# petim0/fly_bProject

Hardware: AMD Instinct MI355X
Metric: env-steps/sec (PPO rollout + update), 8192 envs per GPU (higher is better)
Workload: dtype f32 (optimizer step: fp16x2 operand split; rollout policy + critic: bf16x3 operand split; fp32 accumulate)

## Files before the change

### fly_bproject_amd/csrc/domain_rand.h

```cpp
#ifndef DOMAIN_RAND_H
#define DOMAIN_RAND_H

#include "flyhip.h"
#include "obs_norm.h"

struct DrSlot {
    float* table;
    FlyRandomization r;
};
constexpr unsigned long DR_SLOT = OBS_NORM_SLOT + 16;
constexpr unsigned long DR_CONFIG_BYTES = DR_SLOT + ((sizeof(DrSlot) + 15) & ~15UL);
static_assert(FLY_DR_PARAMS == 6 && FLY_DR_ROW == 8, "a row is m[6] | count | 0: two 16-byte stores");

#ifdef __HIPCC__
__device__ __forceinline__ const DrSlot* dr_slot(const FlyConfig* c)
{
    return reinterpret_cast<const DrSlot*>(reinterpret_cast<const char*>(c) + DR_SLOT);
}

__device__ __forceinline__ uint32_t dr_lowbias32(uint32_t x)
{
    x ^= x >> 16;
    x *= 0x7feb352du;
    x ^= x >> 15;
    x *= 0x846ca68bu;
    x ^= x >> 16;
    return x;
}

__device__ __forceinline__ void dr_draw(const FlyConfig* c, uint32_t e, uint32_t k, float m[FLY_DR_PARAMS])
{
    const DrSlot* s = dr_slot(c);
    const uint32_t key = dr_lowbias32(s->r.seed ^ dr_lowbias32(e));
    const uint32_t ctr = dr_lowbias32(key + k);
#pragma unroll
    for (int j = 0; j < FLY_DR_PARAMS; ++j) {
        const uint32_t h = dr_lowbias32(ctr + 0x9E3779B9u * (uint32_t)(j + 1));
        const float u = __fmul_rn((float)(h >> 8), 5.9604644775390625e-8f);
        const float lo = s->r.lo[j], hi = s->r.hi[j];
        m[j] = __fadd_rn(lo, __fmul_rn(__fsub_rn(hi, lo), u));
    }
}

__device__ __forceinline__ void dr_load_row(const FlyConfig* c, long e, float m[FLY_DR_PARAMS], uint32_t& k)
{
    const float4* row = reinterpret_cast<const float4*>(dr_slot(c)->table + e * FLY_DR_ROW);
    const float4 a = row[0], b = row[1];
    m[0] = a.x; m[1] = a.y; m[2] = a.z; m[3] = a.w; m[4] = b.x; m[5] = b.y;
    k = __builtin_bit_cast(uint32_t, b.z);
}

__device__ __forceinline__ void dr_store_row(const FlyConfig* c, long e, const float m[FLY_DR_PARAMS], uint32_t k)
{
    float4* row = reinterpret_cast<float4*>(dr_slot(c)->table + e * FLY_DR_ROW);
    row[0] = make_float4(m[0], m[1], m[2], m[3]);
    row[1] = make_float4(m[4], m[5], __builtin_bit_cast(float, k), 0.0f);
}
#endif

#endif
```

### fly_bproject_amd/csrc/fly_body.inc

```

constexpr int LANES_PER_ENV = 8;
constexpr int BLOCK = 256;
constexpr int ENVS_PER_BLOCK = BLOCK / LANES_PER_ENV;


template <int CTRL>
__device__ __forceinline__ float dpp_f(float x)
{
    return __builtin_bit_cast(float, __builtin_amdgcn_update_dpp(0, __builtin_bit_cast(int, x), CTRL, 0xF, 0xF, true));
}
template <int CTRL>
__device__ __forceinline__ int dpp_i(int x)
{
    return __builtin_amdgcn_update_dpp(0, x, CTRL, 0xF, 0xF, true);
}
__device__ __forceinline__ float row_sum(float x)
{
    x += dpp_f<0xB1>(x);
    x += dpp_f<0x4E>(x);
    x += dpp_f<0x141>(x);
    return x;
}
__device__ __forceinline__ int row_sum_i(int x)
{
    x += dpp_i<0xB1>(x);
    x += dpp_i<0x4E>(x);
    x += dpp_i<0x141>(x);
    return x;
}
__device__ __forceinline__ float row_get(float x, int src)
{
    return __shfl(x, src, LANES_PER_ENV);
}

__device__ __forceinline__ float dot3(float a0, float a1, float a2, float b0, float b1, float b2)
{
    return fmaf(a0, b0, fmaf(a1, b1, a2 * b2));
}
__device__ __forceinline__ float clampf(float x, float lim) { return fminf(fmaxf(x, -lim), lim); }

struct Root {
    float px, py, pz, qx, qy, qz, qw, vx, vy, vz, wx, wy, wz;
};

__device__ __forceinline__ void quat_rot(const float q[4], float v0, float v1, float v2, float sign, float o[3])
{
    float qw = q[3];
    float s = 2.0f * (qw * qw) - 1.0f;
    float cx = q[1] * v2 - q[2] * v1;
    float cy = q[2] * v0 - q[0] * v2;
    float cz = q[0] * v1 - q[1] * v0;
    float dot = q[0] * v0 + q[1] * v1 + q[2] * v2;
    o[0] = (v0 * s + sign * (cx * qw * 2.0f)) + q[0] * dot * 2.0f;
    o[1] = (v1 * s + sign * (cy * qw * 2.0f)) + q[1] * dot * 2.0f;
    o[2] = (v2 * s + sign * (cz * qw * 2.0f)) + q[2] * dot * 2.0f;
}

__device__ __forceinline__ float py_mod(float a, float b)
{
    float m = fmodf(a, b);
    if (m != 0.0f && ((b < 0.0f) != (m < 0.0f))) m += b;
    return m;
}

struct RootObs {
    float vl[3], wl[3], yaw, roll, pitch, ang, up_proj, heading_proj, pot;
};

__device__ __forceinline__ RootObs root_obs(const FlyConfig* __restrict__ c, const Root& r)
{
    RootObs o;
    const float two_pi = 6.28318530717958647692f;
    float t0 = c->target[0] - r.px, t1 = c->target[1] - r.py, t2 = 0.0f;
    float nrm = sqrtf(t0 * t0 + t1 * t1 + t2 * t2);
    o.pot = -nrm / c->dt;
    float dn = nrm < 1e-9f ? 1e-9f : nrm;
    float d0 = t0 / dn, d1 = t1 / dn, d2 = t2 / dn;
    float x1 = r.qx, y1 = r.qy, z1 = r.qz, w1 = r.qw;
    float x2 = -0.0f, y2 = -0.0f, z2 = -0.0f, w2 = 1.0f;
    float ww = (z1 + x1) * (x2 + y2);
    float yy = (w1 - y1) * (w2 + z2);
    float zz = (w1 + y1) * (w2 - z2);
    float xx = ww + yy + zz;
    float qq = 0.5f * (xx + (z1 - x1) * (x2 - y2));
    float tq[4];
    tq[3] = qq - ww + (z1 - y1) * (y2 - z2);
    tq[0] = qq - xx + (x1 + w1) * (x2 + w2);
    tq[1] = qq - yy + (w1 - x1) * (y2 + z2);
    tq[2] = qq - zz + (z1 + y1) * (w2 - x2);
    float up[3], hd[3];
    quat_rot(tq, 0.0f, 0.0f, 1.0f, 1.0f, up);
    quat_rot(tq, 1.0f, 0.0f, 0.0f, 1.0f, hd);
    o.up_proj = up[2];
    o.heading_proj = hd[0] * d0 + hd[1] * d1 + hd[2] * d2;
    quat_rot(tq, r.vx, r.vy, r.vz, -1.0f, o.vl);
    quat_rot(tq, r.wx, r.wy, r.wz, -1.0f, o.wl);
    float x = tq[0], y = tq[1], z = tq[2], w = tq[3];
    float sinr = 2.0f * (w * x + y * z);
    float cosr = w * w - x * x - y * y + z * z;
    float roll = atan2f(sinr, cosr);
    float sinp = 2.0f * (w * y - z * x);
    float pitch;
    if (fabsf(sinp) >= 1.0f) {
        float sgn = (sinp > 0.0f) ? 1.0f : ((sinp < 0.0f) ? -1.0f : 0.0f);
        pitch = 1.57079632679489661923f * sgn;
    } else {
        pitch = asinf(sinp);
    }
    float siny = 2.0f * (w * z + x * y);
    float cosy = w * w + x * x - y * y - z * z;
    float yaw = atan2f(siny, cosy);
    o.roll = py_mod(roll, two_pi);
    o.pitch = py_mod(pitch, two_pi);
    o.yaw = py_mod(yaw, two_pi);
    float walk = atan2f(c->target[2] - r.pz, c->target[0] - r.px);
    o.ang = walk - o.yaw;
    return o;
}

__device__ __forceinline__ float scale_action(float a, float lo, float hi)
{
    float t = 0.5f * (a + 1.0f);
    t = t * (hi - lo);
    return t + lo;
}

struct FlyRegs {
    Root r;
    float jq[3], jqd[3];
    float pot, prev_pot;
    int rs;
    long progress;
    float dm[FLY_DR_PARAMS];
    uint32_t dk;
};

template <int PH, bool DR = false>
__device__ __forceinline__ void fly_load(FlyRegs& st, const FlyConfig* __restrict__ c, const FlyBuffers& b, const int block)
{
    const int n = c->num_envs;
    const int tid = threadIdx.x;
    const int sub = tid & (LANES_PER_ENV - 1);
    const long e_raw = (long)block * ENVS_PER_BLOCK + tid / LANES_PER_ENV;
    const long e = e_raw < n ? e_raw : (long)(n - 1);
    const bool is_leg = sub < FLY_NUM_LEGS;
    const int j0 = 3 * (is_leg ? sub : 0);
    constexpr bool NEED_ROOT = (PH & (PH_RESET | PH_INTEGRATE | PH_OBS | PH_REWARD)) != 0;
    constexpr bool NEED_DOF = (PH & (PH_RESET | PH_INTEGRATE | PH_OBS)) != 0;
    constexpr bool NEED_POT = (PH & (PH_RESET | PH_OBS | PH_REWARD)) != 0;
    constexpr bool NEED_FLAG = (PH & (PH_RESET | PH_REWARD)) != 0;
    constexpr bool NEED_PROG = (PH & (PH_RESET | PH_REWARD | PH_PROGRESS)) != 0;
    Root r = {};
    if (NEED_ROOT) {
        const float* rp = b.root + e * FLY_ROOT_DIM;
        r.px = rp[0]; r.py = rp[1]; r.pz = rp[2]; r.qx = rp[3]; r.qy = rp[4]; r.qz = rp[5]; r.qw = rp[6];
        r.vx = rp[7]; r.vy = rp[8]; r.vz = rp[9]; r.wx = rp[10]; r.wy = rp[11]; r.wz = rp[12];
    }
    st.r = r;
#pragma unroll
    for (int i = 0; i < 3; ++i) { st.jq[i] = 0.0f; st.jqd[i] = 0.0f; }
    if (NEED_DOF && is_leg) {
        const float* dp = b.dof_state + e * (FLY_NUM_DOF * 2) + 2 * j0;
#pragma unroll
        for (int i = 0; i < 3; ++i) { st.jq[i] = dp[2 * i]; st.jqd[i] = dp[2 * i + 1]; }
    }
    st.pot = 0.0f; st.prev_pot = 0.0f;
    if (NEED_POT) { st.pot = b.pot[e]; st.prev_pot = b.prev_pot[e]; }
    st.rs = 0;
    if (NEED_FLAG) st.rs = (int)(b.reset[e] != 0);
    st.progress = 0;
    if (NEED_PROG) st.progress = b.progress[e];
    if constexpr (DR && (PH & (PH_RESET | PH_INTEGRATE)) != 0) dr_load_row(c, e, st.dm, st.dk);
}

template <int PH, bool DR = false>
__device__ __forceinline__ void fly_body(const FlyConfig* __restrict__ c, const float* __restrict__ actions, const FlyBuffers& b,
                                         float* obs_tile, const int block, const FlyRegs& st, FlyRegs* st_out = nullptr,
                                         const float* actions_tile = nullptr)
{

    const int n = c->num_envs;
    const int tid = threadIdx.x;
    const int sub = tid & (LANES_PER_ENV - 1);
    const int env_in_blk = tid / LANES_PER_ENV;
    const long e_raw = (long)block * ENVS_PER_BLOCK + env_in_blk;
    const bool valid = e_raw < n;
    const long e = valid ? e_raw : (long)(n - 1);
    const bool is_leg = sub < FLY_NUM_LEGS;
    const bool is_abd = sub < FLY_NUM_ABDOMEN;
    const int leg = is_leg ? sub : 0;
    const int abd = is_abd ? sub : 0;
    const int j0 = 3 * leg;

    float lo[3], hi[3], pose[3];
#pragma unroll
    for (int i = 0; i < 3; ++i) { lo[i] = c->dof_lo[j0 + i]; hi[i] = c->dof_hi[j0 + i]; pose[i] = c->dof_pose[j0 + i]; }

    Root r = st.r;
    float jq[3] = {st.jq[0], st.jq[1], st.jq[2]}, jqd[3] = {st.jqd[0], st.jqd[1], st.jqd[2]}, jt[3] = {0, 0, 0};
    float pot = st.pot, prev_pot = st.prev_pot;
    int rs = st.rs;
    long progress = st.progress;
    float dm[FLY_DR_PARAMS];
    uint32_t dk = 0;
    bool drew = false;
    if constexpr (DR) {
#pragma unroll
        for (int j = 0; j < FLY_DR_PARAMS; ++j) dm[j] = st.dm[j];
        dk = st.dk;
    }
    float cf[3] = {0, 0, 0};
    float cfa[3] = {0, 0, 0};

    if (PH & PH_SCALE) {
        if (is_leg) {
            const float* ap = actions_tile ? actions_tile + env_in_blk * FLY_NUM_DOF + j0 : actions + e * FLY_NUM_DOF + j0;
#pragma unroll
            for (int i = 0; i < 3; ++i) jt[i] = scale_action(ap[i], lo[i], hi[i]);
        }
    } else if ((PH & (PH_INTEGRATE | PH_OBS | PH_REWARD)) && is_leg) {
        const float* tp = b.targets + e * FLY_NUM_DOF + j0;
#pragma unroll
        for (int i = 0; i < 3; ++i) jt[i] = tp[i];
    }
    if (!(PH & (PH_INTEGRATE)) && (PH & (PH_OBS | PH_REWARD))) {
        if (is_leg) {
            const float* fp = b.contact + (e * FLY_NUM_CONTACT + FLY_NUM_ABDOMEN + leg) * 3;
            cf[0] = fp[0]; cf[1] = fp[1]; cf[2] = fp[2];
        }
        if (is_abd) {
            const float* fp = b.contact + (e * FLY_NUM_CONTACT + abd) * 3;
            cfa[0] = fp[0]; cfa[1] = fp[1]; cfa[2] = fp[2];
        }
    }

    const bool reset_after = c->reset_after_sim != 0;

    auto do_reset = [&]() {
        if (rs) {
            r.px = 0.0f; r.py = 0.0f; r.pz = c->start_height; r.qx = 0.0f; r.qy = 0.0f; r.qz = 0.0f; r.qw = 1.0f;
            r.vx = r.vy = r.vz = r.wx = r.wy = r.wz = 0.0f;
#pragma unroll
            for (int i = 0; i < 3; ++i) { jq[i] = is_leg ? pose[i] : 0.0f; jqd[i] = 0.0f; }
            float tx = c->target[0] - 0.0f, ty = c->target[1] - 0.0f;
            float nrm = sqrtf(__fadd_rn(__fadd_rn(__fmul_rn(tx, tx), __fmul_rn(ty, ty)), 0.0f));
            float p = -nrm / c->dt;
            prev_pot = p; pot = p;
            rs = 0; progress = 0;
            if constexpr (DR) {
                dr_draw(c, (uint32_t)e, dk, dm);
                dk += 1u;
                drew = true;
            }
        }
    };

    if ((PH & PH_RESET) && !(reset_after && (PH & PH_INTEGRATE))) do_reset();

    if (PH & PH_INTEGRATE) {
        const int nsub = c->substeps;
        const float h = c->dt / (float)nsub;
        const float kp = DR ? __fmul_rn(c->kp, dm[0]) : c->kp, kd = DR ? __fmul_rn(c->kd, dm[1]) : c->kd;
        const float eff = DR ? __fmul_rn(c->effort, dm[2]) : c->effort, vmax = c->vmax, Jinv = 1.0f / c->joint_inertia;
        const float minv = 1.0f / (DR ? __fmul_rn(c->mass, dm[3]) : c->mass), g = DR ? __fmul_rn(c->gravity, dm[5]) : c->gravity;
        const float I0 = DR ? __fmul_rn(c->inertia[0], dm[3]) : c->inertia[0];
        const float I1 = DR ? __fmul_rn(c->inertia[1], dm[3]) : c->inertia[1];
        const float I2 = DR ? __fmul_rn(c->inertia[2], dm[3]) : c->inertia[2];
        const float I0inv = 1.0f / I0, I1inv = 1.0f / I1, I2inv = 1.0f / I2;
        const float vlim = c->max_lin_vel, wlim = c->max_ang_vel;
        const float kc = c->kc, cd = c->cdamp, mu = DR ? __fmul_rn(c->mu, dm[4]) : c->mu, cv = c->cvisc;
        const float Lf = c->femur_len, Lt = c->tibia_len;
        const float ld = 1.0f - h * c->lin_damp, ad = 1.0f - h * c->ang_damp;
        const float att0 = c->leg_attach[leg][0], att1 = c->leg_attach[leg][1], att2 = c->leg_attach[leg][2];
        const float azim = c->leg_azimuth[leg], sg = c->leg_sigma[leg];
        const float ab0 = c->abdomen_pts[abd][0], ab1 = c->abdomen_pts[abd][1], ab2 = c->abdomen_pts[abd][2];
        const float al0 = c->alpha0, be0 = c->beta0;
        const float kc_leg = is_leg ? kc : 0.0f, kc_abd = is_abd ? kc : 0.0f;

        for (int s = 0; s < nsub; ++s) {
#pragma unroll
            for (int i = 0; i < 3; ++i) {
                float tau = fmaf(kp, jt[i] - jq[i], -(kd * jqd[i]));
                tau = fminf(fmaxf(tau, -eff), eff);
                float v = fmaf(h * Jinv, tau, jqd[i]);
                v = fminf(fmaxf(v, -vmax), vmax);
                float x = fmaf(h, v, jq[i]);
                if (x < lo[i]) { x = lo[i]; v = fmaxf(v, 0.0f); }
                if (x > hi[i]) { x = hi[i]; v = fminf(v, 0.0f); }
                jq[i] = x; jqd[i] = v;
            }
            const float qx = r.qx, qy = r.qy, qz = r.qz, qw = r.qw;
            const float R00 = fmaf(-2.0f, fmaf(qy, qy, qz * qz), 1.0f), R01 = 2.0f * fmaf(qx, qy, -(qz * qw)), R02 = 2.0f * fmaf(qx, qz, qy * qw);
            const float R10 = 2.0f * fmaf(qx, qy, qz * qw), R11 = fmaf(-2.0f, fmaf(qx, qx, qz * qz), 1.0f), R12 = 2.0f * fmaf(qy, qz, -(qx * qw));
            const float R20 = 2.0f * fmaf(qx, qz, -(qy * qw)), R21 = 2.0f * fmaf(qy, qz, qx * qw), R22 = fmaf(-2.0f, fmaf(qx, qx, qy * qy), 1.0f);
            float psi = fmaf(sg, jq[0] - pose[0], azim);
            float al = al0 + (jq[1] - pose[1]);
            float gm = al + be0 + (jq[2] - pose[2]);
            float psid = sg * jqd[0], ald = jqd[1], gmd = ald + jqd[2];
            const float sp = __sinf(psi), cp = __cosf(psi);
            const float sa = __sinf(al), ca = __cosf(al);
            const float sgm = __sinf(gm), cg = __cosf(gm);
            float rho = fmaf(Lf, ca, Lt * cg), zeta = fmaf(Lf, sa, Lt * sgm);
            float rhod = -fmaf(Lf * sa, ald, Lt * sgm * gmd);
            float zetad = fmaf(Lf * ca, ald, Lt * cg * gmd);
            float Fx_l = 0.0f, Fy_l = 0.0f, Fz_l = 0.0f, Tx_l = 0.0f, Ty_l = 0.0f, Tz_l = 0.0f;
            auto contact = [&](float rbx, float rby, float rbz, float rdx, float rdy, float rdz, float kc_l, auto moving, float (&f)[3]) {
                constexpr bool MOVING = decltype(moving)::value;
                float rwx = dot3(R00, R01, R02, rbx, rby, rbz);
                float rwy = dot3(R10, R11, R12, rbx, rby, rbz);
                float rwz = dot3(R20, R21, R22, rbx, rby, rbz);
                float d = fmaxf(-(r.pz + rwz), 0.0f);
                float ux = r.vx + fmaf(r.wy, rwz, -(r.wz * rwy));
                float uy = r.vy + fmaf(r.wz, rwx, -(r.wx * rwz));
                float uz = r.vz + fmaf(r.wx, rwy, -(r.wy * rwx));
                if (MOVING) {
                    ux += dot3(R00, R01, R02, rdx, rdy, rdz);
                    uy += dot3(R10, R11, R12, rdx, rdy, rdz);
                    uz += dot3(R20, R21, R22, rdx, rdy, rdz);
                }
                float fn = fmaxf(kc_l * d * fmaf(-cd, uz, 1.0f), 0.0f);
                float ut = __builtin_amdgcn_sqrtf(fmaf(ux, ux, uy * uy));
                float ft = fminf(cv * ut, mu * fn);
                float sc = ft * __builtin_amdgcn_rcpf(ut + 1e-9f);
                float fx = -sc * ux, fy = -sc * uy, fz = fn;
                f[0] = fx; f[1] = fy; f[2] = fz;
                Fx_l += fx; Fy_l += fy; Fz_l += fz;
                Tx_l += fmaf(rwy, fz, -(rwz * fy));
                Ty_l += fmaf(rwz, fx, -(rwx * fz));
                Tz_l += fmaf(rwx, fy, -(rwy * fx));
            };
            contact(fmaf(cp, rho, att0), fmaf(sp, rho, att1), att2 + zeta,
                    fmaf(cp, rhod, -(sp * rho * psid)), fmaf(sp, rhod, cp * rho * psid), zetad, kc_leg, std::true_type{}, cf);
            contact(ab0, ab1, ab2, 0.0f, 0.0f, 0.0f, kc_abd, std::false_type{}, cfa);
            float Fx = row_sum(Fx_l), Fy = row_sum(Fy_l), Fz = row_sum(Fz_l);
            float Tx = row_sum(Tx_l), Ty = row_sum(Ty_l), Tz = row_sum(Tz_l);
            r.vx = clampf(fmaf(h, Fx * minv, r.vx) * ld, vlim);
            r.vy = clampf(fmaf(h, Fy * minv, r.vy) * ld, vlim);
            r.vz = clampf(fmaf(h, fmaf(Fz, minv, g), r.vz) * ld, vlim);
            float wbx = dot3(R00, R10, R20, r.wx, r.wy, r.wz);
            float wby = dot3(R01, R11, R21, r.wx, r.wy, r.wz);
            float wbz = dot3(R02, R12, R22, r.wx, r.wy, r.wz);
            float tbx = dot3(R00, R10, R20, Tx, Ty, Tz);
            float tby = dot3(R01, R11, R21, Tx, Ty, Tz);
            float tbz = dot3(R02, R12, R22, Tx, Ty, Tz);
            float ax = (tbx - fmaf(wby * I2, wbz, -(wbz * I1 * wby))) * I0inv;
            float ay = (tby - fmaf(wbz * I0, wbx, -(wbx * I2 * wbz))) * I1inv;
            float az = (tbz - fmaf(wbx * I1, wby, -(wby * I0 * wbx))) * I2inv;
            wbx = clampf(fmaf(h, ax, wbx) * ad, wlim);
            wby = clampf(fmaf(h, ay, wby) * ad, wlim);
            wbz = clampf(fmaf(h, az, wbz) * ad, wlim);
            r.wx = dot3(R00, R01, R02, wbx, wby, wbz);
            r.wy = dot3(R10, R11, R12, wbx, wby, wbz);
            r.wz = dot3(R20, R21, R22, wbx, wby, wbz);
            r.px = fmaf(h, r.vx, r.px); r.py = fmaf(h, r.vy, r.py); r.pz = fmaf(h, r.vz, r.pz);
            const float hh = 0.5f * h;
            float nqx = fmaf(hh, fmaf(r.wx, qw, fmaf(r.wy, qz, -(r.wz * qy))), qx);
            float nqy = fmaf(hh, fmaf(-r.wx, qz, fmaf(r.wy, qw, r.wz * qx)), qy);
            float nqz = fmaf(hh, fmaf(r.wx, qy, fmaf(-r.wy, qx, r.wz * qw)), qz);
            float nqw = fmaf(hh, -fmaf(r.wx, qx, fmaf(r.wy, qy, r.wz * qz)), qw);
            float inv = __builtin_amdgcn_rsqf(fmaf(nqx, nqx, fmaf(nqy, nqy, fmaf(nqz, nqz, nqw * nqw))));
            r.qx = nqx * inv; r.qy = nqy * inv; r.qz = nqz * inv; r.qw = nqw * inv;
        }
    }

    if ((PH & PH_RESET) && reset_after && (PH & PH_INTEGRATE)) do_reset();

    float touching_f = 0.0f;
    float obs_act[3] = {0, 0, 0};
    float z_obs = 0.0f, heading_proj = 0.0f;
    if (PH & PH_OBS) {
        prev_pot = pot;
        RootObs ro = root_obs(c, r);
        pot = ro.pot;
        float* row = obs_tile + env_in_blk * FLY_NUM_OBS;
        if (sub == LANES_PER_ENV - 1) {
            row[0] = r.pz; row[1] = ro.vl[0]; row[2] = ro.vl[1]; row[3] = ro.vl[2];
            row[4] = ro.wl[0]; row[5] = ro.wl[1]; row[6] = ro.wl[2];
            row[7] = ro.yaw; row[8] = ro.roll; row[9] = ro.ang; row[10] = ro.up_proj; row[11] = ro.heading_proj;
            row[66] = ro.pitch;
        }
        z_obs = r.pz; heading_proj = ro.heading_proj;
        if (is_leg) {
            const float vs = c->dof_vel_scale;
#pragma unroll
            for (int i = 0; i < 3; ++i) {
                float u = __fsub_rn(__fsub_rn(__fmul_rn(2.0f, jq[i]), hi[i]), lo[i]) / __fsub_rn(hi[i], lo[i]);
                row[12 + j0 + i] = u;
                row[30 + j0 + i] = __fmul_rn(jqd[i], vs);
                row[48 + j0 + i] = jt[i];
                obs_act[i] = jt[i];
            }
            float ssum = __fadd_rn(__fadd_rn(cf[0], cf[1]), cf[2]);
            touching_f = ssum > 0.0f ? 1.0f : 0.0f;
            row[67 + leg] = touching_f;
        }
        __syncthreads();
        const long tile_base = (long)block * ENVS_PER_BLOCK * FLY_NUM_OBS;
        const long total = (long)n * FLY_NUM_OBS;
        const float4* src4 = reinterpret_cast<const float4*>(obs_tile);
        const bool aligned16 = (reinterpret_cast<uintptr_t>(b.obs) & 15) == 0;
        for (int i = tid; i < ENVS_PER_BLOCK * FLY_NUM_OBS / 4; i += BLOCK) {
            long g = tile_base + 4L * i;
            if (aligned16 && g + 3 < total) {
                *reinterpret_cast<float4*>(b.obs + g) = src4[i];
            } else {
                for (int k = 0; k < 4; ++k)
                    if (g + k < total) b.obs[g + k] = obs_tile[4 * i + k];
            }
        }
    } else if (PH & PH_REWARD) {
        const float* row = b.obs + e * FLY_NUM_OBS;
        z_obs = row[0]; heading_proj = row[11];
        if (is_leg) {
#pragma unroll
            for (int i = 0; i < 3; ++i) obs_act[i] = row[48 + j0 + i];
        }
    }

    if (PH & PH_PROGRESS) progress += 1;

    float reward = 0.0f;
    if (PH & PH_REWARD) {
        if (progress == 0) progress = 1;
        const float uw = c->up_weight, hw = c->heading_weight;
        float elec = 0.0f, acost = 0.0f;
        int lim = 0, touching = 0;
        if (is_leg) {
#pragma unroll
            for (int i = 0; i < 3; ++i) {
                acost += jt[i] * jt[i];
                elec += fabsf(__fsub_rn(jt[i], obs_act[i]));
                lim += (obs_act[i] > __fmul_rn(hi[i], 0.9f)) ? 1 : 0;
                lim += (obs_act[i] < __fmul_rn(lo[i], 0.9f)) ? 1 : 0;
            }
            touching = (__fadd_rn(__fadd_rn(cf[0], cf[1]), cf[2]) > 0.0f) ? 1 : 0;
        }
        elec = row_sum(elec); acost = row_sum(acost);
        lim = row_sum_i(lim); touching = row_sum_i(touching);
        float bsum = is_abd ? __fadd_rn(__fadd_rn(cfa[0], cfa[1]), cfa[2]) : 0.0f;
        float abd_sum = 0.0f;
#pragma unroll
        for (int k = 0; k < FLY_NUM_ABDOMEN; ++k) abd_sum = __fadd_rn(abd_sum, row_get(bsum, k));
        const float z = z_obs;
        float heading_r = (heading_proj > 0.8f) ? hw : __fmul_rn(hw, heading_proj) / 0.8f;
        float up_r = 0.0f;
        if (z > 1.4f) up_r = __fadd_rn(up_r, uw);
        if (z < 2.1f) up_r = __fsub_rn(up_r, uw);
        float ori = __fadd_rn(__fmul_rn(r.qz, r.qz), __fmul_rn(r.qw, r.qw));
        float orient_r = (ori > 0.98f) ? uw : 0.0f;
        float leg_r = __fmul_rn((float)touching, 0.1f);
        float progress_r = __fsub_rn(pot, prev_pot);
        float total;
        if (c->reward_mode == 0) {
            total = __fadd_rn(0.5f, __fmul_rn(up_r, orient_r));
            total = __fsub_rn(total, __fmul_rn(c->energy_cost_scale, elec));
            total = __fsub_rn(total, __fmul_rn((float)lim, c->joints_at_limit_cost_scale));
            total = __fadd_rn(total, leg_r);
        } else {
            total = __fadd_rn(__fmul_rn(progress_r, 2.0f), 0.5f);
            total = __fadd_rn(total, __fmul_rn(up_r, orient_r));
            total = __fadd_rn(total, heading_r);
            total = __fsub_rn(total, __fmul_rn(c->actions_cost_scale, acost));
            total = __fsub_rn(total, __fmul_rn(c->energy_cost_scale, elec));
            total = __fsub_rn(total, __fmul_rn((float)lim, c->joints_at_limit_cost_scale));
        }
        const bool dead = (z < c->termination_height) || (z > c->termination_height_up) || (ori < 0.5f) || (abd_sum > 0.0f);
        if (dead) total = c->death_cost;
        if (dead || progress >= (long)c->max_episode_length - 1) rs = 1;
        reward = total;
    }

    if (st_out) {
        st_out->r = r;
#pragma unroll
        for (int i = 0; i < 3; ++i) { st_out->jq[i] = jq[i]; st_out->jqd[i] = jqd[i]; }
        st_out->pot = pot; st_out->prev_pot = prev_pot; st_out->rs = rs; st_out->progress = progress;
        if constexpr (DR) {
#pragma unroll
            for (int j = 0; j < FLY_DR_PARAMS; ++j) st_out->dm[j] = dm[j];
            st_out->dk = dk;
        }
    }
    if (!valid) return;
    if constexpr (DR) {
        if (drew && sub == 0) dr_store_row(c, e, dm, dk);
    }
    if (PH & (PH_SCALE)) {
        if (is_leg) {
            float* tp = b.targets + e * FLY_NUM_DOF + j0;
#pragma unroll
            for (int i = 0; i < 3; ++i) tp[i] = jt[i];
        }
    }
    if (PH & (PH_RESET | PH_INTEGRATE)) {
        if (is_leg) {
            float* dp = b.dof_state + e * (FLY_NUM_DOF * 2) + 2 * j0;
#pragma unroll
            for (int i = 0; i < 3; ++i) { dp[2 * i] = jq[i]; dp[2 * i + 1] = jqd[i]; }
        }
        if (sub == LANES_PER_ENV - 1) {
            float* rp = b.root + e * FLY_ROOT_DIM;
            rp[0] = r.px; rp[1] = r.py; rp[2] = r.pz; rp[3] = r.qx; rp[4] = r.qy; rp[5] = r.qz; rp[6] = r.qw;
            rp[7] = r.vx; rp[8] = r.vy; rp[9] = r.vz; rp[10] = r.wx; rp[11] = r.wy; rp[12] = r.wz;
        }
    }
    if (PH & PH_INTEGRATE) {
        if (is_leg) {
            float* fp = b.contact + (e * FLY_NUM_CONTACT + FLY_NUM_ABDOMEN + leg) * 3;
            fp[0] = cf[0]; fp[1] = cf[1]; fp[2] = cf[2];
        }
        if (is_abd) {
            float* fp = b.contact + (e * FLY_NUM_CONTACT + abd) * 3;
            fp[0] = cfa[0]; fp[1] = cfa[1]; fp[2] = cfa[2];
        }
    }
    if (sub == LANES_PER_ENV - 2) {
        if (PH & (PH_RESET | PH_OBS)) { b.pot[e] = pot; b.prev_pot[e] = prev_pot; }
        if (PH & (PH_RESET | PH_REWARD)) b.reset[e] = (int64_t)rs;
        if (PH & (PH_RESET | PH_REWARD | PH_PROGRESS)) b.progress[e] = (int64_t)progress;
        if (PH & PH_REWARD) {
            b.reward[e] = reward;
            if (b.ep_return) {
                const float er = b.ep_return[e] + reward, el = b.ep_length[e] + 1.0f;
                if (rs) {
                    b.done_return[e] += er; b.done_length[e] += el; b.done_count[e] += 1.0f;
                    b.ep_return[e] = 0.0f; b.ep_length[e] = 0.0f;
                } else {
                    b.ep_return[e] = er; b.ep_length[e] = el;
                }
            }
        }
    }
}
// ... 1 lines not shown
```

### fly_bproject_amd/csrc/flyhip_abi.hip

```cpp
#include <hip/hip_runtime.h>
#include <string.h>
#include <stdint.h>
#include <stdio.h>
#include <stdarg.h>
#include <new>
#include "flyhip.h"
#include "obs_norm.h"
#include "domain_rand.h"
#include "launch.h"
#include <math.h>

struct FlyEnv {
    FlyConfig host;
    FlyConfig* dev;
    float* poses;
    const float* obs_norm;
    float* dr_table;
};

namespace {
thread_local char g_err[512] = "";

int fail(int code, const char* fmt, ...)
{
// ... 4 lines not shown
    return code;
}

int hip_fail(hipError_t e, const char* what)
{
    return fail(FLY_E_HIP, "%s: %s", what, hipGetErrorString(e));
}

int check_buffers(const FlyBuffers* b, int phases)
{
    if (!b) return fail(FLY_E_ARG, "FlyBuffers is null");
    const bool need_root = phases & (PH_RESET | PH_INTEGRATE | PH_OBS | PH_REWARD);
    const bool need_dof = phases & (PH_RESET | PH_INTEGRATE | PH_OBS);
    const bool need_tgt = phases & (PH_SCALE | PH_INTEGRATE | PH_OBS | PH_REWARD);
    const bool need_con = phases & (PH_INTEGRATE | PH_OBS | PH_REWARD);
    const bool need_pot = phases & (PH_RESET | PH_OBS | PH_REWARD);
    const bool need_obs = phases & (PH_OBS | PH_REWARD);
    const bool need_flags = phases & (PH_RESET | PH_REWARD | PH_PROGRESS);
    if (need_root && !b->root) return fail(FLY_E_ARG, "root is null");
    if (need_dof && !b->dof_state) return fail(FLY_E_ARG, "dof_state is null");
    if (need_tgt && !b->targets) return fail(FLY_E_ARG, "targets is null");
    if (need_con && !b->contact) return fail(FLY_E_ARG, "contact is null");
    if (need_pot && (!b->pot || !b->prev_pot)) return fail(FLY_E_ARG, "pot/prev_pot is null");
    if (need_obs && !b->obs) return fail(FLY_E_ARG, "obs is null");
    if (need_obs && ((uintptr_t)b->obs & 3)) return fail(FLY_E_ARG, "obs must be 4-byte aligned");
    if ((phases & PH_REWARD) && !b->reward) return fail(FLY_E_ARG, "reward is null");
    if (need_flags && (!b->reset || !b->progress)) return fail(FLY_E_ARG, "reset/progress is null");
    return FLY_OK;
}

int launch(FlyHandle h, int phases, const float* actions, const FlyBuffers* b, void* stream)
{
    if (!h) return fail(FLY_E_ARG, "handle is null");
    if ((phases & PH_SCALE) && !actions) return fail(FLY_E_ARG, "actions is null");
    int rc = check_buffers(b, phases);
    if (rc) return rc;
    hipError_t e = flyhip_launch_env(phases, h->dev, h->host.num_envs, actions, b, stream, h->dr_table != nullptr);
    if (e != hipSuccess) return hip_fail(e, "fly env kernel launch");
    return FLY_OK;
}
}

extern "C" {

const char* fly_last_error(void) { return g_err; }
int fly_abi_version(void) { return FLY_ABI_VERSION; }

int fly_create(const FlyConfig* cfg, FlyHandle* out)
{
    if (!cfg || !out) return fail(FLY_E_ARG, "fly_create: null argument");
    if (cfg->num_envs <= 0) return fail(FLY_E_CONFIG, "num_envs must be > 0 (got %d)", cfg->num_envs);
    if (cfg->substeps <= 0 || cfg->substeps > 1024) return fail(FLY_E_CONFIG, "substeps out of range (%d)", cfg->substeps);
    if (!(cfg->dt > 0.0f)) return fail(FLY_E_CONFIG, "dt must be > 0");
    if (!(cfg->mass > 0.0f) || !(cfg->joint_inertia > 0.0f)) return fail(FLY_E_CONFIG, "mass / joint_inertia must be > 0");
    for (int i = 0; i < 3; ++i)
        if (!(cfg->inertia[i] > 0.0f)) return fail(FLY_E_CONFIG, "inertia[%d] must be > 0", i);
    for (int j = 0; j < FLY_NUM_DOF; ++j)
        if (!(cfg->dof_hi[j] > cfg->dof_lo[j])) return fail(FLY_E_CONFIG, "dof limits of joint %d are not ordered", j);
    if (cfg->reward_mode != 0 && cfg->reward_mode != 1) return fail(FLY_E_CONFIG, "reward_mode must be 0 or 1");
    FlyEnv* h = new (std::nothrow) FlyEnv;
    if (!h) return fail(FLY_E_ARG, "out of host memory");
    h->host = *cfg;
    h->dev = nullptr;
    h->poses = nullptr;
    h->obs_norm = nullptr;
    h->dr_table = nullptr;
    hipError_t e = hipMalloc((void**)&h->dev, DR_CONFIG_BYTES);
    if (e != hipSuccess) { delete h; return hip_fail(e, "hipMalloc(FlyConfig)"); }
    e = hipMemcpy(h->dev, cfg, sizeof(FlyConfig), hipMemcpyHostToDevice);
    if (e == hipSuccess) e = hipMemset(reinterpret_cast<char*>(h->dev) + OBS_NORM_SLOT, 0, DR_CONFIG_BYTES - OBS_NORM_SLOT);
    if (e != hipSuccess) { (void)hipFree(h->dev); delete h; return hip_fail(e, "hipMemcpy(FlyConfig)"); }
    *out = h;
    return FLY_OK;
}

int fly_destroy(FlyHandle h)
{
    if (!h) return fail(FLY_E_ARG, "handle is null");
    hipError_t e = hipFree(h->dev);
    delete h;
    if (e != hipSuccess) return hip_fail(e, "hipFree(FlyConfig)");
    return FLY_OK;
}

int fly_step(FlyHandle h, const float* actions, const FlyBuffers* b, void* stream)
{
    return launch(h, PH_SCALE | PH_RESET | PH_INTEGRATE | PH_OBS | PH_PROGRESS | PH_REWARD, actions, b, stream);
}

int ppo_rollout_step(FlyHandle h, const FlyBuffers* b, const float* params, const float* params_frag, const float* x,
                     const float* eps, const float* var, int32_t var_steps, float var_decay, float var_min,
                     float* act_out, float* logp_out, float* v_out, const uint16_t* params_b3,
                     const int32_t* var_steps_base, void* stream)
{
    if (!h) return fail(FLY_E_ARG, "handle is null");
    if (!params || !params_frag || !x || !eps || !var || !act_out || !logp_out)
        return fail(FLY_E_ARG, "ppo_rollout_step: null pointer");
    if (var_steps < 0 || var_steps > (1 << 20)) return fail(FLY_E_ARG, "ppo_rollout_step: var_steps out of range");
    int rc = check_buffers(b, PH_SCALE | PH_RESET | PH_INTEGRATE | PH_OBS | PH_PROGRESS | PH_REWARD);
    if (rc) return rc;
    hipError_t e = flyhip_launch_rollout_step(h->dev, b, params, params_frag, x, h->host.num_envs, eps, var, var_steps,
                                              var_decay, var_min, act_out, logp_out, v_out, params_b3, var_steps_base, stream,
                                              h->obs_norm != nullptr, h->dr_table != nullptr);
    if (e != hipSuccess) return hip_fail(e, "ppo_rollout_step launch");
    return FLY_OK;
}

static int rollout_all_impl(FlyHandle h, const FlyBuffers* b, const float* params, const float* params_frag, float* obs_ring,
                            const float* eps_all, const float* var, float var_decay, float var_min, float* act_all,
                            float* logp_all, float* v_ring, float* reward_all, int32_t T, const int32_t* rows_applied,
                            const uint16_t* params_b3, int64_t* reset_rows, int64_t* progress_rows, void* stream,
                            unsigned long long* stamps)
{
    if ((reset_rows != nullptr) != (progress_rows != nullptr)) return fail(FLY_E_ARG, "ppo_rollout_all: reset_rows and progress_rows go together");
    if (!h) return fail(FLY_E_ARG, "handle is null");
    if (!params || !params_frag || !obs_ring || !eps_all || !var || !act_all || !logp_all || !v_ring || !reward_all)
        return fail(FLY_E_ARG, "ppo_rollout_all: null pointer");
    if (T <= 0 || T > (1 << 20)) return fail(FLY_E_ARG, "ppo_rollout_all: T out of range");
    if (!b) return fail(FLY_E_ARG, "ppo_rollout_all: buffers are null");
    FlyBuffers bb = *b;
    bb.obs = obs_ring; bb.reward = reward_all;
    int rc = check_buffers(&bb, PH_SCALE | PH_RESET | PH_INTEGRATE | PH_OBS | PH_PROGRESS | PH_REWARD);
    if (rc) return rc;
    if (stamps && h->obs_norm) return fail(FLY_E_ARG, "the stamped rollout does not normalise observations (fly_set_obs_norm)");
    if (stamps && h->dr_table) return fail(FLY_E_ARG, "the stamped rollout does not randomise the physics (fly_set_randomization)");
    hipError_t e = flyhip_launch_rollout_all(h->dev, &bb, params, params_frag, obs_ring, h->host.num_envs, eps_all, var,
                                             var_decay, var_min, act_all, logp_all, v_ring, reward_all, T, rows_applied,
                                             params_b3, reset_rows, progress_rows, stream, stamps, stamps ? nullptr : h->poses,
                                             h->obs_norm != nullptr, h->dr_table != nullptr);
    if (e != hipSuccess) return hip_fail(e, "ppo_rollout_all launch");
    return FLY_OK;
}

int ppo_rollout_all(FlyHandle h, const FlyBuffers* b, const float* params, const float* params_frag, float* obs_ring,
                    const float* eps_all, const float* var, float var_decay, float var_min, float* act_all,
                    float* logp_all, float* v_ring, float* reward_all, int32_t T, const int32_t* rows_applied,
                    const uint16_t* params_b3, int64_t* reset_rows, int64_t* progress_rows, void* stream)
{
    return rollout_all_impl(h, b, params, params_frag, obs_ring, eps_all, var, var_decay, var_min, act_all, logp_all, v_ring,
                            reward_all, T, rows_applied, params_b3, reset_rows, progress_rows, stream, nullptr);
}

extern "C" int flyhip_debug_rollout_all_stamped(FlyHandle h, const FlyBuffers* b, const float* params, const float* params_frag,
                                                float* obs_ring, const float* eps_all, const float* var, float var_decay,
                                                float var_min, float* act_all, float* logp_all, float* v_ring, float* reward_all,
                                                int32_t T, const uint16_t* params_b3, int64_t* reset_rows, int64_t* progress_rows,
                                                unsigned long long* stamps, void* stream)
{
    if (!stamps) return fail(FLY_E_ARG, "stamps is null");
    return rollout_all_impl(h, b, params, params_frag, obs_ring, eps_all, var, var_decay, var_min, act_all, logp_all, v_ring,
                            reward_all, T, nullptr, params_b3, reset_rows, progress_rows, stream, stamps);
}

int fly_set_pose_record(FlyHandle h, float* poses)
{
    if (!h) return fail(FLY_E_ARG, "handle is null");
    if (reinterpret_cast<uintptr_t>(poses) & 3) return fail(FLY_E_ARG, "fly_set_pose_record: poses is not 4-byte aligned");
    h->poses = poses;
    return FLY_OK;
}

int fly_set_obs_norm(FlyHandle h, const float* table)
{
    if (!h) return fail(FLY_E_ARG, "handle is null");
    if (reinterpret_cast<uintptr_t>(table) & 3) return fail(FLY_E_ARG, "fly_set_obs_norm: table is not 4-byte aligned");
    hipError_t e = hipMemcpy(reinterpret_cast<char*>(h->dev) + OBS_NORM_SLOT, &table, sizeof(table), hipMemcpyHostToDevice);
    if (e != hipSuccess) return hip_fail(e, "fly_set_obs_norm");
    h->obs_norm = table;
    return FLY_OK;
}

int fly_set_randomization(FlyHandle h, const FlyRandomization* r, float* env_params, void* stream)
{
    if (!h) return fail(FLY_E_ARG, "handle is null");
    if (!r) {
        h->dr_table = nullptr;
        return FLY_OK;
    }
    static const char* const names[FLY_DR_PARAMS] = {"kp", "kd", "effort", "mass", "mu", "gravity"};
    for (int j = 0; j < FLY_DR_PARAMS; ++j) {
        const float lo = r->lo[j], hi = r->hi[j];
        if (!isfinite(lo) || !isfinite(hi)) return fail(FLY_E_ARG, "fly_set_randomization: %s bounds are not finite", names[j]);
        if (!(lo > 0.0f)) return fail(FLY_E_ARG, "fly_set_randomization: %s lower bound must be > 0 (got %g)", names[j], (double)lo);
        if (lo > hi) return fail(FLY_E_ARG, "fly_set_randomization: %s range is not ordered (%g > %g)", names[j], (double)lo, (double)hi);
    }
    if (!env_params) return fail(FLY_E_ARG, "fly_set_randomization: env_params is null");
    if (reinterpret_cast<uintptr_t>(env_params) & 15) return fail(FLY_E_ARG, "fly_set_randomization: env_params is not 16-byte aligned");
    DrSlot slot;
    slot.table = env_params;
    slot.r = *r;
    hipError_t e = hipMemcpy(reinterpret_cast<char*>(h->dev) + DR_SLOT, &slot, sizeof(slot), hipMemcpyHostToDevice);
    if (e != hipSuccess) return hip_fail(e, "fly_set_randomization");
    e = flyhip_launch_dr_register(h->dev, h->host.num_envs, stream);
    if (e != hipSuccess) return hip_fail(e, "fly_set_randomization launch");
    h->dr_table = env_params;
    return FLY_OK;
}

int ppo_obs_norm_pass(const float* ring, int64_t rows, int64_t count_from, const float* table, float* out, double* sets,
                      void* stream)
{
    if (!ring || !table || !out || !sets) return fail(FLY_E_ARG, "ppo_obs_norm_pass: null pointer");
    if (rows <= 0 || count_from < 0 || count_from > rows) return fail(FLY_E_ARG, "ppo_obs_norm_pass: bad row range");
    if (ring == out) return fail(FLY_E_ARG, "ppo_obs_norm_pass: out must not alias the ring");
    hipError_t e = flyhip_launch_obs_norm_pass(ring, rows, count_from, table, out, sets, stream);
    if (e != hipSuccess) return hip_fail(e, "ppo_obs_norm_pass launch");
    return FLY_OK;
}

int ppo_obs_norm_merge(double* stats, float* table, const double* sets, int64_t k, float clip, void* stream)
{
    if (!stats || !table || !sets) return fail(FLY_E_ARG, "ppo_obs_norm_merge: null pointer");
    if (k <= 0 || !(clip > 0.0f)) return fail(FLY_E_ARG, "ppo_obs_norm_merge: bad argument");
    hipError_t e = flyhip_launch_obs_norm_merge(stats, table, sets, k, clip, stream);
    if (e != hipSuccess) return hip_fail(e, "ppo_obs_norm_merge launch");
    return FLY_OK;
}

int ppo_td_gae_vnorm(const float* reward, const float* v, const float* v_next, const float* done, const float* table,
                     float gamma, float lambda, int64_t T, int64_t N, float* target_out, float* adv_out, double* sets,
                     int mode_flags, void* stream)
{
    if (!reward || !v || !v_next || !done || !table || !target_out || !adv_out || !sets)
        return fail(FLY_E_ARG, "ppo_td_gae_vnorm: null pointer");
    if (T <= 0 || N <= 0) return fail(FLY_E_ARG, "ppo_td_gae_vnorm: T and N must be > 0");
    if (reinterpret_cast<uintptr_t>(sets) & 7) return fail(FLY_E_ARG, "ppo_td_gae_vnorm: sets is not 8-byte aligned");
    if ((mode_flags & PPO_GAE_SCAN) && (mode_flags & PPO_GAE_MASK_RECURRENCE))
        return fail(FLY_E_ARG, "ppo_td_gae_vnorm: PPO_GAE_SCAN does not implement the masked recurrence");
    hipError_t e = flyhip_launch_td_gae_vnorm(reward, v, v_next, done, table, gamma, lambda, T, N, target_out, adv_out, sets,
                                              mode_flags, stream);
    if (e != hipSuccess) return hip_fail(e, "ppo_td_gae_vnorm launch");
    return FLY_OK;
}

int ppo_value_norm_merge(const double* stats_in, const double* sets, int64_t k, double* stats_out, float* table_out, void* stream)
{
    if (!stats_in || !sets || !stats_out || !table_out) return fail(FLY_E_ARG, "ppo_value_norm_merge: null pointer");
    if (k <= 0) return fail(FLY_E_ARG, "ppo_value_norm_merge: k must be > 0");
    if ((reinterpret_cast<uintptr_t>(stats_in) | reinterpret_cast<uintptr_t>(sets) | reinterpret_cast<uintptr_t>(stats_out)) & 7)
        return fail(FLY_E_ARG, "ppo_value_norm_merge: a float64 buffer is not 8-byte aligned");
    if (stats_in < stats_out + FLY_VALUE_NORM_SET && stats_out < stats_in + FLY_VALUE_NORM_SET)
        return fail(FLY_E_ARG, "ppo_value_norm_merge: stats_out must not overlap stats_in");
    hipError_t e = flyhip_launch_value_norm_merge(stats_in, sets, k, stats_out, table_out, stream);
    if (e != hipSuccess) return hip_fail(e, "ppo_value_norm_merge launch");
    return FLY_OK;
}

int ppo_value_norm_apply(const float* target, int64_t n, const float* table, float* out, void* stream)
{
    if (!target || !table || !out) return fail(FLY_E_ARG, "ppo_value_norm_apply: null pointer");
    if (n <= 0) return fail(FLY_E_ARG, "ppo_value_norm_apply: n must be > 0");
    if (target < out + n && out < target + n) return fail(FLY_E_ARG, "ppo_value_norm_apply: out must not alias the targets");
    hipError_t e = flyhip_launch_value_norm_apply(target, n, table, out, stream);
    if (e != hipSuccess) return hip_fail(e, "ppo_value_norm_apply launch");
    return FLY_OK;
}

int ppo_lambda_targets(const float* adv, const float* v, const float* table, int64_t n, float* target_out, double* sets,
                       void* stream)
{
    if (!adv || !v || !target_out) return fail(FLY_E_ARG, "ppo_lambda_targets: null pointer");
    if (n < 0) return fail(FLY_E_ARG, "ppo_lambda_targets: n must be >= 0");
    if ((reinterpret_cast<uintptr_t>(adv) | reinterpret_cast<uintptr_t>(v) | reinterpret_cast<uintptr_t>(table) |
         reinterpret_cast<uintptr_t>(target_out)) & 3)
        return fail(FLY_E_ARG, "ppo_lambda_targets: a float32 buffer is not 4-byte aligned");
    if (reinterpret_cast<uintptr_t>(sets) & 7) return fail(FLY_E_ARG, "ppo_lambda_targets: sets is not 8-byte aligned");
    if ((target_out < adv + n && adv < target_out + n) || (target_out < v + n && v < target_out + n))
        return fail(FLY_E_ARG, "ppo_lambda_targets: target_out must not alias the inputs");
    if (n == 0 && !sets) return FLY_OK;
    hipError_t e = flyhip_launch_lambda_targets(adv, v, table, n, target_out, sets, stream);
    if (e != hipSuccess) return hip_fail(e, "ppo_lambda_targets launch");
    return FLY_OK;
}

static int check_episodic(const char* what, bool any_null, int64_t max_episode_length, int64_t T, int64_t N, int mode_flags)
{
    if (any_null) return fail(FLY_E_ARG, "%s: null pointer", what);
    if (T <= 0 || N <= 0) return fail(FLY_E_ARG, "%s: T and N must be > 0", what);
    if (max_episode_length <= 0) return fail(FLY_E_ARG, "%s: max_episode_length must be > 0", what);
    if (mode_flags != 0 && mode_flags != PPO_GAE_SCAN)
        return fail(FLY_E_ARG, "%s: mode_flags must be 0 or PPO_GAE_SCAN (got %d)", what, mode_flags);
    return FLY_OK;
}

int ppo_td_gae_episodic(const float* reward, const float* v, const float* v_next, const int64_t* reset, const int64_t* progress,
                        const int64_t* ended_prev, int64_t max_episode_length, float gamma, float lambda, int64_t T, int64_t N,
                        float* target_out, float* adv_out, int mode_flags, void* stream)
{
    int rc = check_episodic("ppo_td_gae_episodic",
                            !reward || !v || !v_next || !reset || !progress || !ended_prev || !target_out || !adv_out,
                            max_episode_length, T, N, mode_flags);
    if (rc) return rc;
    hipError_t e = flyhip_launch_td_gae_episodic(reward, v, v_next, reset, progress, ended_prev, max_episode_length, gamma, lambda,
                                                 T, N, target_out, adv_out, mode_flags, stream);
    if (e != hipSuccess) return hip_fail(e, "ppo_td_gae_episodic launch");
    return FLY_OK;
}

int ppo_td_gae_episodic_vnorm(const float* reward, const float* v, const float* v_next, const int64_t* reset,
                              const int64_t* progress, const int64_t* ended_prev, int64_t max_episode_length, const float* table,
                              float gamma, float lambda, int64_t T, int64_t N, float* target_out, float* adv_out, double* sets,
                              int mode_flags, void* stream)
{
    int rc = check_episodic("ppo_td_gae_episodic_vnorm",
                            !reward || !v || !v_next || !reset || !progress || !ended_prev || !table || !target_out || !adv_out || !sets,
                            max_episode_length, T, N, mode_flags);
// ... 529 lines not shown
```

Before: 70.36 million.

## Split root observation math across lanes and skip abdomen contact when idle

Root observation work (four quaternion rotations and three atan2 calls), previously done redundantly on all eight lanes of an env, is now spread so each lane computes one rotation and one angle, with shuffles to share heading and yaw and per-lane writes of the observation entries. The abdomen contact evaluation is skipped for a whole wavefront when a ballot shows no lane has abdomen penetration, with a debug word to force the old path. Clamps use the fmed3 builtin. The aim is to cut redundant transcendental and contact ALU work in the substep loop, at the cost of extra select logic and a ballot per substep.

```diff
diff --git a/fly_bproject_amd/csrc/domain_rand.h b/fly_bproject_amd/csrc/domain_rand.h
--- a/fly_bproject_amd/csrc/domain_rand.h
+++ b/fly_bproject_amd/csrc/domain_rand.h
@@ -9,6 +9,8 @@
     FlyRandomization r;
 };
 constexpr unsigned long DR_SLOT = OBS_NORM_SLOT + 16;
+constexpr unsigned long ENV_DEBUG_SLOT = OBS_NORM_SLOT + 8;
+static_assert(ENV_DEBUG_SLOT + sizeof(int32_t) <= DR_SLOT, "the debug word sits between the table pointer and the DR slot");
 constexpr unsigned long DR_CONFIG_BYTES = DR_SLOT + ((sizeof(DrSlot) + 15) & ~15UL);
 static_assert(FLY_DR_PARAMS == 6 && FLY_DR_ROW == 8, "a row is m[6] | count | 0: two 16-byte stores");
 
@@ -16,6 +18,11 @@
 __device__ __forceinline__ const DrSlot* dr_slot(const FlyConfig* c)
 {
     return reinterpret_cast<const DrSlot*>(reinterpret_cast<const char*>(c) + DR_SLOT);
+}
+
+__device__ __forceinline__ int32_t env_debug_word(const FlyConfig* c)
+{
+    return *reinterpret_cast<const int32_t*>(reinterpret_cast<const char*>(c) + ENV_DEBUG_SLOT);
 }
 
 __device__ __forceinline__ uint32_t dr_lowbias32(uint32_t x)
diff --git a/fly_bproject_amd/csrc/fly_body.inc b/fly_bproject_amd/csrc/fly_body.inc
--- a/fly_bproject_amd/csrc/fly_body.inc
+++ b/fly_bproject_amd/csrc/fly_body.inc
@@ -37,7 +37,7 @@
 {
     return fmaf(a0, b0, fmaf(a1, b1, a2 * b2));
 }
-__device__ __forceinline__ float clampf(float x, float lim) { return fminf(fmaxf(x, -lim), lim); }
+__device__ __forceinline__ float clampf(float x, float lim) { return __builtin_amdgcn_fmed3f(x, -lim, lim); }
 
 struct Root {
     float px, py, pz, qx, qy, qz, qw, vx, vy, vz, wx, wy, wz;
@@ -64,10 +64,11 @@
 }
 
 struct RootObs {
-    float vl[3], wl[3], yaw, roll, pitch, ang, up_proj, heading_proj, pot;
+    float rot[3], eul, ang;
+    float heading_proj, pot;
 };
 
-__device__ __forceinline__ RootObs root_obs(const FlyConfig* __restrict__ c, const Root& r)
+__device__ __forceinline__ RootObs root_obs(const FlyConfig* __restrict__ c, const Root& r, const int sub)
 {
     RootObs o;
     const float two_pi = 6.28318530717958647692f;
@@ -88,17 +89,15 @@
     tq[0] = qq - xx + (x1 + w1) * (x2 + w2);
     tq[1] = qq - yy + (w1 - x1) * (y2 + z2);
     tq[2] = qq - zz + (z1 + y1) * (w2 - x2);
-    float up[3], hd[3];
-    quat_rot(tq, 0.0f, 0.0f, 1.0f, 1.0f, up);
-    quat_rot(tq, 1.0f, 0.0f, 0.0f, 1.0f, hd);
-    o.up_proj = up[2];
-    o.heading_proj = hd[0] * d0 + hd[1] * d1 + hd[2] * d2;
-    quat_rot(tq, r.vx, r.vy, r.vz, -1.0f, o.vl);
-    quat_rot(tq, r.wx, r.wy, r.wz, -1.0f, o.wl);
+    const bool l0 = sub == 0, l1 = sub == 1, l2 = sub == 2;
+    const float v0 = l0 ? 0.0f : (l1 ? 1.0f : (l2 ? r.vx : r.wx));
+    const float v1 = (l0 || l1) ? 0.0f : (l2 ? r.vy : r.wy);
+    const float v2 = l0 ? 1.0f : (l1 ? 0.0f : (l2 ? r.vz : r.wz));
+    quat_rot(tq, v0, v1, v2, sub < 2 ? 1.0f : -1.0f, o.rot);
+    o.heading_proj = row_get(o.rot[0] * d0 + o.rot[1] * d1 + o.rot[2] * d2, 1);
     float x = tq[0], y = tq[1], z = tq[2], w = tq[3];
     float sinr = 2.0f * (w * x + y * z);
     float cosr = w * w - x * x - y * y + z * z;
-    float roll = atan2f(sinr, cosr);
     float sinp = 2.0f * (w * y - z * x);
     float pitch;
     if (fabsf(sinp) >= 1.0f) {
@@ -109,12 +108,11 @@
     }
     float siny = 2.0f * (w * z + x * y);
     float cosy = w * w + x * x - y * y - z * z;
-    float yaw = atan2f(siny, cosy);
-    o.roll = py_mod(roll, two_pi);
-    o.pitch = py_mod(pitch, two_pi);
-    o.yaw = py_mod(yaw, two_pi);
-    float walk = atan2f(c->target[2] - r.pz, c->target[0] - r.px);
-    o.ang = walk - o.yaw;
+    const float ay = l1 ? siny : (l2 ? c->target[2] - r.pz : sinr);
+    const float ax = l1 ? cosy : (l2 ? c->target[0] - r.px : cosr);
+    const float a = atan2f(ay, ax);
+    o.eul = py_mod(sub < 2 ? a : pitch, two_pi);
+    o.ang = a - row_get(o.eul, 1);
     return o;
 }
 
@@ -276,14 +274,15 @@
         const float ab0 = c->abdomen_pts[abd][0], ab1 = c->abdomen_pts[abd][1], ab2 = c->abdomen_pts[abd][2];
         const float al0 = c->alpha0, be0 = c->beta0;
         const float kc_leg = is_leg ? kc : 0.0f, kc_abd = is_abd ? kc : 0.0f;
+        const bool abd_always = env_debug_word(c) != 0;
 
         for (int s = 0; s < nsub; ++s) {
 #pragma unroll
             for (int i = 0; i < 3; ++i) {
                 float tau = fmaf(kp, jt[i] - jq[i], -(kd * jqd[i]));
-                tau = fminf(fmaxf(tau, -eff), eff);
+                tau = clampf(tau, eff);
                 float v = fmaf(h * Jinv, tau, jqd[i]);
-                v = fminf(fmaxf(v, -vmax), vmax);
+                v = clampf(v, vmax);
                 float x = fmaf(h, v, jq[i]);
                 if (x < lo[i]) { x = lo[i]; v = fmaxf(v, 0.0f); }
                 if (x > hi[i]) { x = hi[i]; v = fminf(v, 0.0f); }
@@ -331,7 +330,13 @@
             };
             contact(fmaf(cp, rho, att0), fmaf(sp, rho, att1), att2 + zeta,
                     fmaf(cp, rhod, -(sp * rho * psid)), fmaf(sp, rhod, cp * rho * psid), zetad, kc_leg, std::true_type{}, cf);
-            contact(ab0, ab1, ab2, 0.0f, 0.0f, 0.0f, kc_abd, std::false_type{}, cfa);
+            const float rwz_b = dot3(R20, R21, R22, ab0, ab1, ab2);
+            const float d_b = fmaxf(-(r.pz + rwz_b), 0.0f);
+            if (abd_always || __builtin_amdgcn_ballot_w64(kc_abd * d_b != 0.0f) != 0) {
+                contact(ab0, ab1, ab2, 0.0f, 0.0f, 0.0f, kc_abd, std::false_type{}, cfa);
+            } else {
+                cfa[0] = 0.0f; cfa[1] = 0.0f; cfa[2] = 0.0f;
+            }
             float Fx = row_sum(Fx_l), Fy = row_sum(Fy_l), Fz = row_sum(Fz_l);
             float Tx = row_sum(Tx_l), Ty = row_sum(Ty_l), Tz = row_sum(Tz_l);
             r.vx = clampf(fmaf(h, Fx * minv, r.vx) * ld, vlim);
@@ -370,15 +375,17 @@
     float z_obs = 0.0f, heading_proj = 0.0f;
     if (PH & PH_OBS) {
         prev_pot = pot;
-        RootObs ro = root_obs(c, r);
+        RootObs ro = root_obs(c, r, sub);
         pot = ro.pot;
         float* row = obs_tile + env_in_blk * FLY_NUM_OBS;
-        if (sub == LANES_PER_ENV - 1) {
-            row[0] = r.pz; row[1] = ro.vl[0]; row[2] = ro.vl[1]; row[3] = ro.vl[2];
-            row[4] = ro.wl[0]; row[5] = ro.wl[1]; row[6] = ro.wl[2];
-            row[7] = ro.yaw; row[8] = ro.roll; row[9] = ro.ang; row[10] = ro.up_proj; row[11] = ro.heading_proj;
-            row[66] = ro.pitch;
-        }
+        const bool l0 = sub == 0, l1 = sub == 1, l2 = sub == 2;
+        const int ib = l0 ? 10 : (l1 ? 11 : (l2 ? 1 : 4));
+        if (sub < 4) {
+            row[l0 ? 8 : (l1 ? 7 : (l2 ? 9 : 66))] = l2 ? ro.ang : ro.eul;
+            row[ib] = l0 ? ro.rot[2] : (l1 ? ro.heading_proj : ro.rot[0]);
+        }
+        if (sub == 2 || sub == 3) { row[ib + 1] = ro.rot[1]; row[ib + 2] = ro.rot[2]; }
+        if (sub == 4) row[0] = r.pz;
         z_obs = r.pz; heading_proj = ro.heading_proj;
         if (is_leg) {
             const float vs = c->dof_vel_scale;
diff --git a/fly_bproject_amd/csrc/flyhip_abi.hip b/fly_bproject_amd/csrc/flyhip_abi.hip
--- a/fly_bproject_amd/csrc/flyhip_abi.hip
+++ b/fly_bproject_amd/csrc/flyhip_abi.hip
@@ -180,6 +180,15 @@
                             reward_all, T, nullptr, params_b3, reset_rows, progress_rows, stream, stamps);
 }
 
+extern "C" int flyhip_debug_set_abdomen_pass(FlyHandle h, int always)
+{
+    if (!h) return fail(FLY_E_ARG, "handle is null");
+    const int32_t word = always != 0;
+    hipError_t e = hipMemcpy(reinterpret_cast<char*>(h->dev) + ENV_DEBUG_SLOT, &word, sizeof(word), hipMemcpyHostToDevice);
+    if (e != hipSuccess) return hip_fail(e, "flyhip_debug_set_abdomen_pass");
+    return FLY_OK;
+}
+
 int fly_set_pose_record(FlyHandle h, float* poses)
 {
     if (!h) return fail(FLY_E_ARG, "handle is null");
```

Measured after the change: 71.02 million, median of 6. No clear change (+0.9%).
